# submission2019/cnn-quantization

Hardware: NVIDIA H100
Metric: resnet50_w4a4_images_per_s (higher is better)
Workload: dtype f32

## Files before the change

cnn-quantization_b200/_lib.py:

```python
import ctypes
import os

HERE = os.path.dirname(os.path.abspath(__file__))
LIB_PATH = os.environ.get("FQB200_LIB") or os.path.join(HERE, "libfqb200.so")

OK, ERR_INVALID, ERR_WORKSPACE, ERR_CUDA, ERR_UNSUPPORTED = 0, 1, 2, 3, 4
SCOPE_GROUP, SCOPE_GROUP_MEAN, SCOPE_TENSOR = 0, 1, 2
RANGE_MINMAX, RANGE_LAPLACE, RANGE_GAUS, RANGE_KSTD, RANGE_GIVEN = 0, 1, 2, 3, 4
LEAF_TORCH, LEAF_COMPILED, LEAF_MIDTREAD = 0, 1, 2
PRIOR_STD, PRIOR_B = 0, 1
STATS_STRIDE = 12
STAT_COLUMNS = ("min", "max", "mean", "b", "std", "delta", "offset", "bits", "scale", "zero_point", "qmax", "flags")

ABI_VERSION = 3


class Desc(ctypes.Structure):
    _fields_ = [
        ("outer", ctypes.c_int64), ("groups", ctypes.c_int64), ("inner", ctypes.c_int64),
        ("scope", ctypes.c_int32), ("range_mode", ctypes.c_int32), ("leaf", ctypes.c_int32),
        ("num_bits", ctypes.c_int32), ("positive", ctypes.c_int32), ("solve_f64", ctypes.c_int32),
        ("clip_k", ctypes.c_float),
        ("bit_alloc", ctypes.c_int32), ("bit_alloc_prior", ctypes.c_int32), ("bit_alloc_round", ctypes.c_int32),
        ("bit_alloc_target", ctypes.c_float),
        ("mt_target", ctypes.c_float), ("mt_clip", ctypes.c_int32),
        ("bias_corr", ctypes.c_int32), ("var_corr", ctypes.c_int32), ("stats_only", ctypes.c_int32),
        ("out_stats", ctypes.c_void_p),
        ("bias", ctypes.c_void_p),
        ("bias_period", ctypes.c_int64),
        ("channels_last", ctypes.c_int32),
        ("out_hist", ctypes.c_void_p),
        ("hist_bins", ctypes.c_int32), ("hist_offset", ctypes.c_int32),
        ("out_hist_clamped", ctypes.c_void_p),
        ("relu_passthrough", ctypes.c_int32),
        ("residual", ctypes.c_void_p), ("residual_relu", ctypes.c_int32),
        ("residual_stats", ctypes.c_void_p), ("residual_bias", ctypes.c_void_p),
        ("pool", ctypes.c_int32), ("pool_h", ctypes.c_int64), ("pool_w", ctypes.c_int64), ("pool_out", ctypes.c_void_p),
        ("given_delta", ctypes.c_void_p), ("given_offset", ctypes.c_void_p), ("given_bits", ctypes.c_void_p),
        ("debug_stamps", ctypes.c_void_p),
    ]


_vp, _i64, _i32, _f32, _sz, _desc = (ctypes.c_void_p, ctypes.c_int64, ctypes.c_int, ctypes.c_float, ctypes.c_size_t,
                                      ctypes.POINTER(Desc))
PROTOTYPES = {
    "fqb200_abi_version": (_i32, []),
    "fqb200_last_error": (ctypes.c_char_p, []),
    "fqb200_resident_ctas": (_i32, []),
    "fqb200_plan_info": (_i32, [_desc, ctypes.POINTER(ctypes.c_int64)]),
    "fqb200_selftest_division": (_i32, [_vp, _vp, _vp, _vp, _i64, _vp]),
    "fqb200_workspace_bytes": (_sz, [_desc]),
    "fqb200_workspace_init": (_i32, [_vp, _sz, _vp]),
    "fqb200_float2gemmlowp": (_i32, [_vp, _vp, _i64, _f32, _f32, _i32, _i32, _i32, _vp, _vp]),
    "fqb200_quantize1": (_i32, [_vp, _vp, _vp, _i64, _i64, _i64, _vp, _vp, _vp, _i32, _i32, _vp, _i32, _vp]),
    "fqb200_quantize1_bca": (_i32, [_vp, _vp, _i64, _i64, _i64, _vp, _vp, _vp, _i32, _i32, _vp, _i32, _vp, _vp, _sz, _vp]),
    "fqb200_fused": (_i32, [_desc, _vp, _vp, _vp, _sz, _vp]),
    "fqb200_fused_into": (_i32, [_desc, _vp, _vp, _i64, _vp, _sz, _vp]),
    "fqb200_add_relu": (_i32, [_vp, _vp, _vp, _i64, _vp]),
    "fqb200_maxpool2d_nhwc": (_i32, [_vp, _vp, _i64, _i64, _i64, _i64, _i32, _i32, _i32, _i32, _i32, _i32, _vp]),
    "fqb200_maxpool2d_nhwc_into": (_i32, [_vp, _vp, _i64, _i64, _i64, _i64, _i32, _i32, _i32, _i32, _i32, _i32, _i64, _vp]),
    "fqb200_kld_threshold": (_i32, [_vp, _i64, _i64, _i32, _i32, _vp, _vp, _vp, _vp, _sz, _vp]),
    "fqb200_kld_workspace_bytes": (_sz, [_i64, _i32]),
    "fqb200_sample_sumsq": (_i32, [_vp, _i64, _i64, _vp, _vp, _sz, _vp]),
    "fqb200_sample_sumsq_workspace_bytes": (_sz, [_i64, _i64]),
    "fqb200_clip_error": (_i32, [_vp, _i64, _i64, _i64, _i32, _vp, _i32, _i32, _i32, _i32, _vp, _vp, _vp, _sz, _i32, _vp]),
    "fqb200_clip_error_workspace_bytes": (_sz, [_i64, _i64, _i64, _i32]),
    "fqb200_clip_mse": (_i32, [_vp, _i64, _i64, _i64, _i32, _vp, _i32, _i32, _i32, _i32, _i32, _vp, _i32, _vp, _vp, _vp, _sz,
                               _i32, _vp]),
    "fqb200_clip_mse_widths": (_i32, [_vp, _i64, _i64, _i64, _i32, _vp, _i32, _i32, _i32, _i32, _i32, _vp, _vp, _i32, _vp, _vp,
                                      _vp, _sz, _i32, _vp]),
    "fqb200_clip_mse_workspace_bytes": (_sz, [_i64, _i64, _i64, _i32, _i32]),
    "fqb200_clip_mse_grid": (_i32, [_vp, _i64, _i64, _i64, _i32, _vp, _i32, _i32, _i32, _i32, _i32, _vp, _i32, _vp, _i32, _vp,
                                    _vp, _vp, _sz, _i32, _vp]),
    "fqb200_clip_mse_grid_workspace_bytes": (_sz, [_i64, _i64, _i64, _i32, _i32, _i32]),
    "fqb200_kmeans1d": (_i32, [_vp, _i64, _i32, _i64, _vp, _i32, _vp, _i32, _i64, _vp, _vp, _vp, _vp, _vp, _vp, _vp, _vp, _sz,
                               _i32, _vp]),
    "fqb200_kmeans1d_workspace_bytes": (_sz, [_i64, _i32]),
    "fqb200_sample_angles": (_i32, [_vp, _i64, _i64, _vp, _vp, _vp, _sz, _i32, _vp]),
    "fqb200_sample_angles_workspace_bytes": (_sz, [_i64, _i64]),
    "fqb200_sample_noise": (_i32, [_vp, _vp, _vp, _i64, _i64, _i64, _vp, _vp, _sz, _i32, _vp]),
    "fqb200_sample_noise_workspace_bytes": (_sz, [_i64, _i64]),
    "fqb200_quantize_weights_given": (_i32, [_vp, _vp, _i64, _i64, _vp, _vp, _vp, _i32, _i32, _i32, _vp, _vp, _sz, _vp]),
    "fqb200_quantize_weights_given_workspace_bytes": (_sz, [_i64, _i64, _i32, _i32, _i32, _i32]),
    "fqb200_allocate_widths": (_i32, [_vp, _i64, ctypes.c_double, _vp, _vp, _vp, _sz, _vp]),
    "fqb200_allocate_widths_workspace_bytes": (_sz, [_i64, ctypes.c_double]),
}
SYMBOLS = tuple(PROTOTYPES)


class FqError(RuntimeError):
    pass


_lib = None


def load():
    global _lib
    if _lib is not None:
        return _lib
    if not os.path.exists(LIB_PATH):
        raise FqError("libfqb200.so is not built (run `python cnn-quantization_b200/build.py` or "
                      "__graft_entry__.build()); there is no CPU fallback for the fake-quantization path")
    lib = ctypes.CDLL(LIB_PATH)
    for name, (restype, argtypes) in PROTOTYPES.items():
        fn = getattr(lib, name)
        fn.restype, fn.argtypes = restype, argtypes
    if lib.fqb200_abi_version() != ABI_VERSION:
        raise FqError("libfqb200.so ABI version mismatch")
    _lib = lib
    return lib


def check(rc):
    if rc != OK:
        raise FqError("fqb200 error %d: %s" % (rc, load().fqb200_last_error().decode()))
```

cnn-quantization_b200/csrc/fq_bulk.cuh:

```cuda
#pragma once
#include <cuda_runtime.h>
#include <stdint.h>

#include "fq_device.cuh"

namespace fqb {

constexpr int kConsumers = kThreads;
constexpr int kBulkThreads = kConsumers + 32;
constexpr int kConsumerWarps = kConsumers / 32;
#ifndef FQB_STAGE_VEC
#define FQB_STAGE_VEC 4
#endif
#ifndef FQB_STAGES
#define FQB_STAGES 6
#endif
#ifndef FQB_BULK_CTAS
#define FQB_BULK_CTAS 1
#endif
constexpr int kBulkCtasPerSm = FQB_BULK_CTAS;
constexpr int kStageVec = FQB_STAGE_VEC;
constexpr int kStages = FQB_STAGES;
constexpr unsigned kStageBytes = kStageVec * kConsumers * 16u;
#ifndef FQB_BULK_SPLIT
#define FQB_BULK_SPLIT 1
#endif
constexpr unsigned kBulkSplit = FQB_BULK_SPLIT;

__device__ __forceinline__ void consumer_sync() { cta_sync(); }

__device__ __forceinline__ unsigned smem_u32(const void* p) { return static_cast<unsigned>(__cvta_generic_to_shared(p)); }
__device__ __forceinline__ void mbar_init(unsigned bar, unsigned count) {
  asm volatile("mbarrier.init.shared::cta.b64 [%0], %1;" ::"r"(bar), "r"(count) : "memory");
}
__device__ __forceinline__ void mbar_fence_init() { asm volatile("fence.mbarrier_init.release.cluster;" ::: "memory"); }
__device__ __forceinline__ void mbar_arrive(unsigned bar) {
  asm volatile("{ .reg .b64 st; mbarrier.arrive.shared::cta.b64 st, [%0]; }" ::"r"(bar) : "memory");
}
__device__ __forceinline__ void mbar_arrive_expect_tx(unsigned bar, unsigned bytes) {
  asm volatile("{ .reg .b64 st; mbarrier.arrive.expect_tx.shared::cta.b64 st, [%0], %1; }" ::"r"(bar), "r"(bytes) : "memory");
}
__device__ __forceinline__ bool mbar_try_wait(unsigned bar, unsigned parity) {
  unsigned ok;
  asm volatile(
      "{ .reg .pred p; mbarrier.try_wait.parity.shared::cta.b64 p, [%1], %2; selp.u32 %0, 1, 0, p; }"
      : "=r"(ok)
      : "r"(bar), "r"(parity)
      : "memory");
  return ok != 0;
}
__device__ __forceinline__ void mbar_wait(unsigned bar, unsigned parity) {
  while (!mbar_try_wait(bar, parity)) {
  }
}
__device__ __forceinline__ void bulk_load_one(unsigned dst_smem, const void* src, unsigned bytes, unsigned bar) {
  asm volatile("cp.async.bulk.shared::cluster.global.mbarrier::complete_tx::bytes [%0], [%1], %2, [%3];" ::"r"(dst_smem),
               "l"(src), "r"(bytes), "r"(bar)
               : "memory");
}
__device__ __forceinline__ void bulk_load(unsigned dst_smem, const void* src, unsigned bytes, unsigned bar) {
  if (kBulkSplit == 1u) {
    bulk_load_one(dst_smem, src, bytes, bar);
    return;
  }
  constexpr unsigned piece = kStageBytes / kBulkSplit;
  for (unsigned off = 0; off < bytes; off += piece)
    bulk_load_one(dst_smem + off, static_cast<const unsigned char*>(src) + off, min(piece, bytes - off), bar);
}

struct FlatGeo {
  unsigned total_v;
  unsigned stride;
  unsigned stage_v;
  unsigned n_stages;
  unsigned unit_stages;
  unsigned units;
  unsigned channels;
  unsigned cv;
};

struct StageMeta {
  unsigned start;
  unsigned count;
  unsigned tag;
  unsigned pad;
};

struct BulkRing {
  alignas(8) unsigned long long full[kStages];
  alignas(8) unsigned long long empty[kStages];
  StageMeta meta[kStages];
  unsigned nstages;
};

struct RingPos {
  unsigned slot, parity, n;
  __device__ __forceinline__ void init(unsigned nstages = kStages) {
    slot = 0;
    parity = 0;
    n = nstages;
  }
  __device__ __forceinline__ void next() {
    if (++slot == n) {
      slot = 0;
      parity ^= 1u;
    }
  }
};

__device__ __forceinline__ void ring_init(BulkRing& r, unsigned nstages = kStages) {
  if (threadIdx.x == 0) {
    r.nstages = nstages;
#pragma unroll
    for (int s = 0; s < kStages; ++s) {
      mbar_init(smem_u32(&r.full[s]), 1u);
      mbar_init(smem_u32(&r.empty[s]), kConsumerWarps);
    }
    mbar_fence_init();
  }
  __syncthreads();
}

struct TicketPlan {
  unsigned nstatic;
  unsigned first, step;
  unsigned dyn_base;
};

constexpr unsigned kPairOffset = kStageBytes / 2u;

__device__ __forceinline__ FlatGeo half_geo(const FlatGeo& g) {
  FlatGeo h = g;
  h.stage_v = (kStageVec / 2u) * g.stride;
  h.n_stages = (g.total_v + h.stage_v - 1u) / h.stage_v;
  h.unit_stages = 2u * g.unit_stages;
  return h;
}

template <bool REV, bool PAIR = false>
__device__ __forceinline__ void produce_phase(const FlatGeo& g, const float4* src, unsigned* counter, const TicketPlan tp,
                                              BulkRing& r, unsigned char* stage_base, RingPos& pos,
                                              const float4* src2 = nullptr) {
  const unsigned total = g.units;
  unsigned k = 0;
  auto fetch = [&]() -> unsigned {
    unsigned long long t;
    if (k < tp.nstatic)
      t = tp.first + static_cast<unsigned long long>(k) * tp.step;
    else
      t = static_cast<unsigned long long>(tp.dyn_base) + atomicAdd(counter, 1u);
    ++k;
    return t < total ? static_cast<unsigned>(t) : 0xffffffffu;
  };
  unsigned cur = fetch();
  unsigned nxt = (cur != 0xffffffffu) ? fetch() : 0xffffffffu;
  while (cur != 0xffffffffu) {
    const unsigned nxt2 = (nxt != 0xffffffffu) ? fetch() : 0xffffffffu;
    const unsigned u = REV ? total - 1u - cur : cur;
    const unsigned g0 = u * g.unit_stages;
    const unsigned g1 = min(g0 + g.unit_stages, g.n_stages);
    for (unsigned i = g0; i < g1; ++i) {
      const unsigned st = REV ? g1 - 1u - (i - g0) : i;
      const unsigned start = st * g.stage_v;
      const unsigned count = min(g.stage_v, g.total_v - start);
      mbar_wait(smem_u32(&r.empty[pos.slot]), pos.parity ^ 1u);
      r.meta[pos.slot].start = start;
      r.meta[pos.slot].count = count;
      r.meta[pos.slot].tag = 0u;
      const unsigned bar = smem_u32(&r.full[pos.slot]);
      mbar_arrive_expect_tx(bar, PAIR ? count * 32u : count * 16u);
      bulk_load(smem_u32(stage_base + pos.slot * kStageBytes), src + start, count * 16u, bar);
      if (PAIR) bulk_load(smem_u32(stage_base + pos.slot * kStageBytes + kPairOffset), src2 + start, count * 16u, bar);
      pos.next();
    }
    cur = nxt;
    nxt = nxt2;
  }
  mbar_wait(smem_u32(&r.empty[pos.slot]), pos.parity ^ 1u);
  r.meta[pos.slot].start = 0u;
  r.meta[pos.slot].count = 0u;
  mbar_arrive(smem_u32(&r.full[pos.slot]));
  pos.next();
}

struct RowsGeo {
  unsigned rows, row_v;
  unsigned stages_per_row;
  unsigned units_per_row;
};

__device__ __forceinline__ RowsGeo half_rows(const FlatGeo& h, const RowsGeo& rg) {
  RowsGeo r = rg;
  r.stages_per_row = (rg.row_v + h.stage_v - 1u) / h.stage_v;
  r.units_per_row = (r.stages_per_row + h.unit_stages - 1u) / h.unit_stages;
  return r;
}

template <bool REV, bool PAIR = false>
__device__ __forceinline__ void produce_rows_phase(const FlatGeo& g, const RowsGeo& rg, const float4* src, unsigned* counter,
                                                   const TicketPlan tp, BulkRing& r, unsigned char* stage_base, RingPos& pos,
                                                   const float4* src2 = nullptr) {
  const unsigned total = g.units;
  unsigned k = 0;
  auto fetch = [&]() -> unsigned {
    unsigned long long t;
    if (k < tp.nstatic)
      t = tp.first + static_cast<unsigned long long>(k) * tp.step;
    else
      t = static_cast<unsigned long long>(tp.dyn_base) + atomicAdd(counter, 1u);
    ++k;
    return t < total ? static_cast<unsigned>(t) : 0xffffffffu;
  };
  unsigned cur = fetch();
  unsigned nxt = (cur != 0xffffffffu) ? fetch() : 0xffffffffu;
  while (cur != 0xffffffffu) {
    const unsigned nxt2 = (nxt != 0xffffffffu) ? fetch() : 0xffffffffu;
    const unsigned u = REV ? total - 1u - cur : cur;
    const unsigned row = u / rg.units_per_row;
    const unsigned part = u - row * rg.units_per_row;
    const unsigned s0 = part * g.unit_stages;
    const unsigned s1 = min(s0 + g.unit_stages, rg.stages_per_row);
    for (unsigned i = s0; i < s1; ++i) {
      const unsigned st = REV ? s1 - 1u - (i - s0) : i;
      const unsigned off = st * g.stage_v;
      const unsigned start = row * rg.row_v + off;
      const unsigned count = min(g.stage_v, rg.row_v - off);
      mbar_wait(smem_u32(&r.empty[pos.slot]), pos.parity ^ 1u);
      r.meta[pos.slot].start = start;
      r.meta[pos.slot].count = count;
      r.meta[pos.slot].tag = row | (i + 1u == s1 ? 0x80000000u : 0u);
      const unsigned bar = smem_u32(&r.full[pos.slot]);
      mbar_arrive_expect_tx(bar, PAIR ? count * 32u : count * 16u);
      bulk_load(smem_u32(stage_base + pos.slot * kStageBytes), src + start, count * 16u, bar);
      if (PAIR) bulk_load(smem_u32(stage_base + pos.slot * kStageBytes + kPairOffset), src2 + start, count * 16u, bar);
      pos.next();
    }
    cur = nxt;
    nxt = nxt2;
  }
  mbar_wait(smem_u32(&r.empty[pos.slot]), pos.parity ^ 1u);
  r.meta[pos.slot].start = 0u;
  r.meta[pos.slot].count = 0u;
  r.meta[pos.slot].tag = 0u;
  mbar_arrive(smem_u32(&r.full[pos.slot]));
  pos.next();
// ... 272 lines not shown
```

cnn-quantization_b200/csrc/fq_cl.cuh:

```cuda
#pragma once

namespace fqb {

__device__ __forceinline__ unsigned enc_ordered(float x) {
  const unsigned b = __float_as_uint(x);
  return (b & 0x80000000u) ? ~b : (b | 0x80000000u);
}
__device__ __forceinline__ float dec_ordered(unsigned e) {
  return __uint_as_float((e & 0x80000000u) ? (e & 0x7fffffffu) : ~e);
}

constexpr unsigned kAccU = 2u * kMaxNhwcChannels;
constexpr unsigned kAccD = 3u * kMaxNhwcChannels;

struct ClView {
  unsigned* amin_inv;
  unsigned* amax;
  double* asum;
  double* asq;
  double* aabs;
};
__device__ __forceinline__ ClView cl_view(const FusedArgs& A, unsigned bank) {
  ClView v;
  v.amin_inv = A.amin_inv + bank * kAccU;
// ... 553 lines not shown
  cl_combine_add_f64(cx.cbuf, g.cv, g.stride, s2.sa, acc.aabs + rb, s2.sa, nullptr, s2.sa, nullptr);
}

template <int LEAF, bool HIST>
__device__ __noinline__ void cl_phase_apply(const FusedArgs& A, ClCtx& cx, const LeafParam (&lp)[4], unsigned* hist) {
  const FlatGeo& g = *cx.g;
  const unsigned t = threadIdx.x;
  if (HIST) {
    for (unsigned i = t; i < kHistWords; i += kConsumers) hist[i] = 0u;
    consumer_sync();
  }
  ClApply<LEAF, HIST> ap{A, hist};
  ap.init(cx.c0, cx.active, lp);
  RingPos pos = cx.pos;
  if (A.pool.tiles) {
    if (A.pool.kind == 3u)
      consume_pool3_phase(g, A.pool, *cx.ring, cx.stages, pos, ap);
    else
      consume_pool_phase(g, A.pool, *cx.ring, cx.stages, pos, ap);
  } else if (A.residual) {
    const FlatGeo h = half_geo(g);
    consume_pair_phase(h, *cx.ring, cx.stages, pos, ap);
  } else {
    consume_phase(g, *cx.ring, cx.stages, pos, ap);
  }
  cx.pos = pos;
  if (HIST) {
    consumer_sync();
    const unsigned bins = static_cast<unsigned>(A.hist_bins);
    const unsigned copies = max(1u, min(static_cast<unsigned>(kWarps), kHistWords / bins));
    for (unsigned b = t; b < bins; b += kConsumers) {
      unsigned long long cnt = 0;
      for (unsigned w = 0; w < copies; ++w) cnt += hist[w * bins + b];
      if (cnt) atomicAdd(A.hist + b, cnt);
    }
    if (LEAF == FQB200_LEAF_MIDTREAD && A.hist_clamped && cx.active) {
#pragma unroll
      for (int i = 0; i < 4; ++i) {
        if (ap.nlo[i]) atomicAdd(A.hist_clamped + 2u * (cx.c0 + i), static_cast<unsigned long long>(ap.nlo[i]));
        if (ap.nhi[i]) atomicAdd(A.hist_clamped + 2u * (cx.c0 + i) + 1u, static_cast<unsigned long long>(ap.nhi[i]));
      }
    }
  }
}

constexpr unsigned kClStagingBytes = 4u * kConsumers * 8u;
constexpr unsigned kClTableChannels = 1024;
constexpr unsigned kClCombineBytes = kClStagingBytes + kClTableChannels * 4u;

template <int LEAF, bool DEV, bool HIST>
__global__ void __launch_bounds__(kBulkThreads, kBulkCtasPerSm) fq_cl_kernel(const __grid_constant__ FusedArgs A) {
  extern __shared__ __align__(128) unsigned char fq_dyn[];
  unsigned char* stages = fq_dyn;
  unsigned char* cbuf = fq_dyn + kStages * kStageBytes;
  float* tab_mean = reinterpret_cast<float*>(cbuf + kClStagingBytes);
  unsigned* hist = reinterpret_cast<unsigned*>(stages + (kStages - 1) * kStageBytes);
  __shared__ BulkRing ring;
  __shared__ LeaderSmem lsm;
  __shared__ alignas(8) unsigned long long solver_done;
  const FlatGeo& g = A.flat;
  const unsigned C = g.channels, cv = g.cv;
  const unsigned launch = ld_ws(&A.sync->launch_count);
  const unsigned bank = launch & 1u;
  const unsigned tag = launch + 1u;
  const bool alloc = (LEAF == FQB200_LEAF_MIDTREAD) || (A.bit_alloc && A.num_bits <= 4);
  const bool aux_needs_b = alloc && LEAF != FQB200_LEAF_MIDTREAD && A.prior == FQB200_PRIOR_B;
  const bool solver_in_s2 = alloc && !aux_needs_b && DEV && gridDim.x > 1u;
  __shared__ alignas(8) unsigned long long phase_go[2];
  if (threadIdx.x == 0) {
    mbar_init(smem_u32(&solver_done), 1u);
    mbar_init(smem_u32(&phase_go[0]), 1u);
    mbar_init(smem_u32(&phase_go[1]), 1u);
  }
  const unsigned nstages = HIST ? kStages - 1u : kStages;
  ring_init(ring, nstages);

  if (threadIdx.x >= kConsumers) {
    if (threadIdx.x == kConsumers) {
      RingPos pos;
      pos.init(nstages);
      const float4* src = reinterpret_cast<const float4*>(A.in);
      const TicketPlan all = {2u, blockIdx.x, gridDim.x, 2u * gridDim.x};
      const TicketPlan no0 = {blockIdx.x == 0 ? 0u : 2u, blockIdx.x - 1u, gridDim.x - 1u, 2u * (gridDim.x - 1u)};
      produce_phase<false>(g, src, &A.sync->unit_counter[0], all, ring, stages, pos);
      if (DEV) {
        mbar_wait(smem_u32(&phase_go[0]), 0u);
        if (solver_in_s2 && blockIdx.x == 0) mbar_wait(smem_u32(&solver_done), 0u);
        produce_phase<true>(g, src, &A.sync->unit_counter[1], solver_in_s2 ? no0 : all, ring, stages, pos);
      }
      if (!A.stats_only) {
        mbar_wait(smem_u32(&phase_go[1]), 0u);
        if (A.pool.tiles && A.pool.kind == 3u)
          produce_pool3_phase(g, A.pool, src, &A.sync->unit_counter[2], all, ring, stages, pos);
        else if (A.pool.tiles)
          produce_pool_phase(g, A.pool, src, &A.sync->unit_counter[2], all, ring, stages, pos);
        else if (A.residual)
          produce_phase<!DEV, true>(half_geo(g), src, &A.sync->unit_counter[2], all, ring, stages, pos,
                                    reinterpret_cast<const float4*>(A.residual));
        else
          produce_phase<!DEV>(g, src, &A.sync->unit_counter[2], all, ring, stages, pos);
      }
    }
    return;
  }

  const unsigned t = threadIdx.x;
  const bool active = t < g.stride;
  const bool direct = cv == g.stride;
  const unsigned col = active ? t % cv : 0u;
  const unsigned c0 = 4u * col;
  const double n = A.n_per_group;
  const ClView acc = cl_view(A, bank);
  const unsigned rep = A.nhwc_rep;
  const unsigned rep_base = (blockIdx.x % rep) * C;
  unsigned epoch = 0;
  if (blockIdx.x == 0) stamp(A, 0);

  if (blockIdx.x == gridDim.x - 1u) {
    const ClView other = cl_view(A, bank ^ 1u);
    uint4* zu = reinterpret_cast<uint4*>(other.amin_inv);
    uint4* zd = reinterpret_cast<uint4*>(other.asum);
    const uint4 z = make_uint4(0u, 0u, 0u, 0u);
    for (unsigned i = t; i < kAccU / 4u; i += kConsumers) zu[i] = z;
    for (unsigned i = t; i < kAccD / 2u; i += kConsumers) zd[i] = z;
  }

  ClCtx cx;
  cx.g = &g;
  cx.ring = &ring;
  cx.stages = stages;
  cx.cbuf = cbuf;
  cx.pos.init(nstages);
  cx.acc = acc;
  cx.rep_base = rep_base;
  cx.c0 = c0;
  cx.active = active;
  float kshift[4];
  cl_phase_s1(A, cx, kshift);
  if (t == 0) mbar_arrive(smem_u32(&phase_go[DEV ? 0 : 1]));
  if (blockIdx.x == 0) stamp(A, 1);
  grid_barrier_cl(A.sync, epoch);
  if (blockIdx.x == 0) stamp(A, 4);

  float mean[4];
  if (direct) {
#pragma unroll
    for (int i = 0; i < 4; ++i)
      mean[i] = static_cast<float>(cl_mean(acc, rep, C, c0 + i, kshift[i], (A.bias && active) ? __ldg(A.bias + c0 + i) : 0.f, n));
  } else {
    for (unsigned c = t; c < C; c += kConsumers)
      tab_mean[c] = static_cast<float>(cl_mean(acc, rep, C, c, ld_tensor(A.in + c), A.bias ? __ldg(A.bias + c) : 0.f, n));
    consumer_sync();
#pragma unroll
    for (int i = 0; i < 4; ++i) mean[i] = tab_mean[c0 + i];
  }

  if (alloc && !aux_needs_b && blockIdx.x == 0) {
    cl_solve_aux(A, acc, lsm, tag, false, !solver_in_s2);
    stamp(A, 12);
    if (t == 0) mbar_arrive(smem_u32(&solver_done));
  }

  if constexpr (DEV) {
    cl_phase_s2(A, cx, mean);
    if (t == 0) mbar_arrive(smem_u32(&phase_go[1]));
    if (blockIdx.x == 0) stamp(A, 5);
    grid_barrier_cl(A.sync, epoch);
    if (blockIdx.x == 0) stamp(A, 8);
    if (aux_needs_b && blockIdx.x == 0) cl_solve_aux(A, acc, lsm, tag, true, true);
  }
  if (alloc && !solver_in_s2) {
    if (t == 0)
      while (ld_acquire_u32(&A.sync->aux_ready) != tag) __nanosleep(40);
    consumer_sync();
  }

  LeafParam lp[4];
  const bool do_export = A.out_stats != nullptr && blockIdx.x == 0;
  if (direct) {
#pragma unroll
    for (int i = 0; i < 4; ++i) lp[i] = cl_channel_param<LEAF, DEV>(A, acc, rep, C, c0 + i, mean[i], n, alloc, do_export && active);
  } else {
    LeafParam* tab_lp = reinterpret_cast<LeafParam*>(cbuf);
// ... 612 lines not shown
```

cnn-quantization_b200/csrc/fqb200.cu:

```cuda
#include <cuda_runtime.h>
#include <math.h>
#include <stdint.h>
#include <stdio.h>
#include <stdlib.h>
#include <string.h>

#include "../../include/fqb200.h"
#include "fq_device.cuh"
#include "fq_bulk.cuh"

namespace fqb {

__constant__ float kGaus[9] = {0.f, 1.24f, 1.71f, 2.15f, 2.55f, 2.93f, 3.28f, 3.61f, 3.92f};
__constant__ float kGausPos[9] = {0.f, 1.71f, 2.15f, 2.55f, 2.93f, 3.28f, 3.61f, 3.92f, 4.2f};
__constant__ float kLaplace[9] = {1.05f, 1.86f, 2.83f, 3.89f, 5.03f, 6.2f, 7.41f, 8.64f, 9.89f};
__constant__ float kLaplacePos[9] = {1.86f, 2.83f, 3.89f, 5.02f, 6.2f, 7.41f, 8.64f, 9.89f, 11.16f};
constexpr int kTable = 101;
__constant__ double kOmegaTable[kTable];
__constant__ double kAlphaTable[kTable];

enum : int { FLAG_PASSTHROUGH = 1, FLAG_TRUE_ZERO = 2, FLAG_RELU = 4 };

struct alignas(16) LeafParam {
  float a, b, c;
// ... 1380 lines not shown

struct Plan {
  fqb::Geometry geo;
  fqb::FlatGeo flat;
  int vec;
  int mode;
  int grid;
};

constexpr uint64_t kUnitsPerCta = 8;

int make_plan(int64_t outer, int64_t groups, int64_t inner, bool can_vec, bool allow_bundle, int max_ctas, Plan* pl) {
  if (outer <= 0 || groups <= 0 || inner <= 0) return fail(FQB200_ERR_INVALID, "non-positive tensor extent%s");
  if (groups > 0x3fffffffLL || outer > 0x7fffffffLL || inner > 0x7fffffffLL * 4LL)
    return fail(FQB200_ERR_UNSUPPORTED, "tensor extent exceeds 2^31%s");
  int vec = (can_vec && inner % 4 == 0) ? 4 : 1;
  int mode = vec;
  uint64_t bundle = 1;
  if (vec == 1 && can_vec && allow_bundle && inner >= 4) {
    const uint64_t b = (inner % 2 == 0) ? 2 : 4;
    const uint64_t row_v = b * static_cast<uint64_t>(inner) / 4;
    if (groups % b == 0 && row_v <= static_cast<uint64_t>(fqb::kThreads)) {
      bundle = b;
      vec = 4;
      mode = 8;
    }
  }
  const uint64_t G = static_cast<uint64_t>(groups) / bundle;
  const uint64_t inner_v = bundle * static_cast<uint64_t>(inner) / vec;
  if (inner_v > 0xffffffffULL) return fail(FQB200_ERR_UNSUPPORTED, "row too long%s");
  const uint64_t stride = (mode == 8) ? (fqb::kThreads / inner_v) * inner_v : fqb::kThreads;
  const uint64_t group_v = static_cast<uint64_t>(outer) * inner_v;
  const uint64_t total_v = group_v * G;
  if (total_v >= (1ULL << 32)) return fail(FQB200_ERR_UNSUPPORTED, "tensors of 2^32 vectors (64 GB) and more are not supported%s");
  const uint64_t ctas = static_cast<uint64_t>(max_ctas);
  const uint64_t min_unit_v = static_cast<uint64_t>(fqb::kRingDepth) * stride;
  uint64_t parts = (kUnitsPerCta * ctas + G - 1) / G;
  const uint64_t max_parts = group_v / min_unit_v > 0 ? group_v / min_unit_v : 1;
  if (parts > max_parts) parts = max_parts;
  if (parts < 1) parts = 1;
  while ((group_v + parts - 1) / parts >= 0x7fffffffULL) ++parts;
  uint64_t part_v = (group_v + parts - 1) / parts;
  if (mode == 8) part_v = (part_v + inner_v - 1) / inner_v * inner_v;
  parts = (group_v + part_v - 1) / part_v;
  if (parts * G >= 0xfffffff0ULL) return fail(FQB200_ERR_UNSUPPORTED, "too many work units%s");
  const uint64_t units = parts * G;
  unsigned lanes = 32;
  while (lanes > 1 && (static_cast<uint64_t>(fqb::kThreads / lanes) < static_cast<uint64_t>(groups) || (lanes >> 1) >= parts)) lanes >>= 1;
  fqb::Geometry& g = pl->geo;
  g.groups = static_cast<unsigned>(G);
  g.channels = static_cast<unsigned>(groups);
  g.bundle = static_cast<unsigned>(bundle);
  g.stride = static_cast<unsigned>(stride);
  g.parts = static_cast<unsigned>(parts);
  g.units = static_cast<unsigned>(units);
  g.inner_v = static_cast<unsigned>(inner_v);
  g.step_q = static_cast<unsigned>(stride / inner_v);
  g.step_r = static_cast<unsigned>(stride % inner_v);
  g.red_lanes = lanes;
  g.part_v = static_cast<unsigned>(part_v);
  g.group_v = group_v;
  g.row_pitch = G * inner_v;
  pl->vec = vec;
  pl->mode = mode;
  pl->grid = grid_for(units, ctas);
  return FQB200_OK;
}

bool flat_eligible(int64_t channels) { return channels % 4 == 0 && channels / 4 >= 1 && channels / 4 <= fqb::kConsumers; }

int make_plan_flat(uint64_t elems, int64_t channels, int max_ctas, Plan* pl) {
  if (elems == 0 || elems % 4 != 0) return fail(FQB200_ERR_UNSUPPORTED, "flat stream needs a multiple of 4 elements%s");
  const uint64_t total_v = elems / 4;
  if (total_v >= (1ULL << 32)) return fail(FQB200_ERR_UNSUPPORTED, "tensors of 2^32 vectors (64 GB) and more are not supported%s");
  const uint64_t cv = channels > 0 ? static_cast<uint64_t>(channels) / 4 : 1;
  if (channels > 0 && !flat_eligible(channels)) return fail(FQB200_ERR_UNSUPPORTED, "channels-last needs C %% 4 == 0 and C <= 2048%s");
  const uint64_t stride = (fqb::kConsumers / cv) * cv;
  const uint64_t stage_v = static_cast<uint64_t>(fqb::kStageVec) * stride;
  const uint64_t n_stages = (total_v + stage_v - 1) / stage_v;
  const uint64_t ctas = static_cast<uint64_t>(max_ctas);
  uint64_t unit_stages = n_stages / (kUnitsPerCta * ctas);
  if (unit_stages < 2) unit_stages = 2;
  if (unit_stages > 64) unit_stages = 64;
  const uint64_t units = (n_stages + unit_stages - 1) / unit_stages;
  fqb::FlatGeo& g = pl->flat;
  g.total_v = static_cast<unsigned>(total_v);
  g.stride = static_cast<unsigned>(stride);
  g.stage_v = static_cast<unsigned>(stage_v);
  g.n_stages = static_cast<unsigned>(n_stages);
  g.unit_stages = static_cast<unsigned>(unit_stages);
  g.units = static_cast<unsigned>(units);
  g.channels = static_cast<unsigned>(channels > 0 ? channels : 0);
  g.cv = static_cast<unsigned>(cv);
  memset(&pl->geo, 0, sizeof(pl->geo));
  pl->geo.channels = g.channels;
  pl->vec = 4;
  pl->mode = 2;
  pl->grid = grid_for(units, ctas);
  return FQB200_OK;
}

int make_plan_rows(uint64_t rows, uint64_t row_elems, int64_t channels, int max_ctas, Plan* pl, fqb::RowsGeo* rg) {
  if (rows == 0 || row_elems == 0 || row_elems % 4 != 0 || rows > fqb::kMaxNhwcChannels)
    return fail(FQB200_ERR_UNSUPPORTED, "row stream needs rows <= 4096 of a multiple of 4 elements%s");
  const uint64_t row_v = row_elems / 4;
  if (rows * row_v >= (1ULL << 32)) return fail(FQB200_ERR_UNSUPPORTED, "tensors of 2^32 vectors (64 GB) and more are not supported%s");
  const uint64_t cv = channels > 0 ? static_cast<uint64_t>(channels) / 4 : 1;
  if (channels > 0 && (!flat_eligible(channels) || row_v % cv != 0)) return fail(FQB200_ERR_UNSUPPORTED, "bias period does not fit the rows%s");
  const uint64_t stride = (fqb::kConsumers / cv) * cv;
  const uint64_t stage_v = static_cast<uint64_t>(fqb::kStageVec) * stride;
  const uint64_t spr = (row_v + stage_v - 1) / stage_v;
  const uint64_t ctas = static_cast<uint64_t>(max_ctas);
  uint64_t unit_stages = rows * spr / (kUnitsPerCta * ctas);
  if (unit_stages < 1) unit_stages = 1;
  if (unit_stages > 64) unit_stages = 64;
  if (unit_stages > spr) unit_stages = spr;
  const uint64_t upr = (spr + unit_stages - 1) / unit_stages;
  const uint64_t units = rows * upr;
  if (units >= 0xfffffff0ULL) return fail(FQB200_ERR_UNSUPPORTED, "too many work units%s");
  fqb::FlatGeo& g = pl->flat;
  g.total_v = static_cast<unsigned>(rows * row_v);
  g.stride = static_cast<unsigned>(stride);
  g.stage_v = static_cast<unsigned>(stage_v);
  g.n_stages = static_cast<unsigned>(rows * spr);
  g.unit_stages = static_cast<unsigned>(unit_stages);
  g.units = static_cast<unsigned>(units);
  g.channels = static_cast<unsigned>(channels > 0 ? channels : 0);
  g.cv = static_cast<unsigned>(cv);
  rg->rows = static_cast<unsigned>(rows);
  rg->row_v = static_cast<unsigned>(row_v);
  rg->stages_per_row = static_cast<unsigned>(spr);
  rg->units_per_row = static_cast<unsigned>(upr);
  memset(&pl->geo, 0, sizeof(pl->geo));
  pl->geo.channels = static_cast<unsigned>(rows);
  pl->vec = 4;
  pl->mode = 3;
  pl->grid = grid_for(units, ctas);
  return FQB200_OK;
}

bool rows_supported(const fqb200_desc* d, bool can_vec) {
  if (d->leaf != FQB200_LEAF_COMPILED || d->range_mode != FQB200_RANGE_MINMAX || d->bias_corr || d->var_corr || d->channels_last ||
      d->out_hist || !can_vec || d->outer != 1 || d->inner % 4 != 0 || d->groups > static_cast<int64_t>(fqb::kMaxNhwcChannels))
    return false;
  if (!(d->scope == FQB200_SCOPE_GROUP_MEAN || d->scope == FQB200_SCOPE_TENSOR || d->groups == 1)) return false;
  if (d->bias) {
    if (d->bias_period >= 0) return false;
    const int64_t c = -d->bias_period;
    if (!flat_eligible(c) || d->inner % c != 0) return false;
  }
  return true;
}

size_t align_up(size_t v, size_t a) { return (v + a - 1) / a * a; }

size_t kld_workspace(int64_t rows, int num_bins) {
  return align_up(static_cast<size_t>(rows) * 4, 256) + static_cast<size_t>(rows) * static_cast<size_t>(num_bins) * 4;
}

size_t sums_workspace(int64_t rows, int64_t row_len, int sums) {
  const unsigned long long chunk = fqb::sums_chunk(static_cast<unsigned long long>(row_len));
  const unsigned long long chunks = (static_cast<unsigned long long>(row_len) + chunk - 1) / chunk;
  return chunks > 1 ? static_cast<size_t>(rows) * static_cast<size_t>(chunks) * static_cast<size_t>(sums) * 8 : 0;
}

template <int S>
int launch_sums(const float* y, const float* q, const float* bias, int64_t bias_period, int64_t rows, int64_t row_len,
                double* out, void* workspace, int32_t max_ctas, void* stream, const char* what) {
  using namespace fqb;
  DeviceInfo* di = nullptr;
  const int rc = get_device(&di);
  if (rc != FQB200_OK) return rc;
  cudaStream_t st = static_cast<cudaStream_t>(stream);
  SumsArgs A;
  memset(&A, 0, sizeof(A));
  A.y = y;
  A.q = q;
  A.bias = bias;
  A.period = static_cast<unsigned>(bias_period < 0 ? 0ull - static_cast<unsigned long long>(bias_period)
                                                   : static_cast<unsigned long long>(bias_period));
  A.rows = static_cast<unsigned long long>(rows);
  A.row_len = static_cast<unsigned long long>(row_len);
  A.chunk = sums_chunk(A.row_len);
  A.chunks = (A.row_len + A.chunk - 1) / A.chunk;
  A.partial = static_cast<double*>(workspace);
  A.out = out;
  const int grid = grid_for(A.rows * A.chunks, di->sms * (2048ull / kSumsThreads), max_ctas);
  const bool vec = row_len % 4 == 0 && aligned16(y) && (!q || aligned16(q));
#define FQB_LAUNCH_SUMS(B)                                                          \
  do {                                                                              \
    if (vec) fq_sums_partial_kernel<4, S, B><<<grid, kSumsThreads, 0, st>>>(A);     \
    else     fq_sums_partial_kernel<1, S, B><<<grid, kSumsThreads, 0, st>>>(A);     \
  } while (0)
  if constexpr (S == 1) FQB_LAUNCH_SUMS(kSumsBiasNone);
  else if (!bias) FQB_LAUNCH_SUMS(kSumsBiasNone);
  else if (bias_period > 0) FQB_LAUNCH_SUMS(kSumsBiasNchw);
  else FQB_LAUNCH_SUMS(kSumsBiasCl);
#undef FQB_LAUNCH_SUMS
  if (A.chunks > 1) {
    const unsigned long long blocks = (A.rows * S + kSumsThreads - 1) / kSumsThreads;
    fq_sums_finish_kernel<S><<<static_cast<unsigned>(blocks), kSumsThreads, 0, st>>>(A);
  }
  return launched(what);
}

size_t angle_workspace(int64_t rows, int64_t row_len) {
  const fqb::AngleSplit s = fqb::angle_split(static_cast<unsigned long long>(rows), static_cast<unsigned long long>(row_len));
  return static_cast<size_t>(s.pairs * s.slices) * fqb::kAngTile * fqb::kAngTile * 8;
}

unsigned long long cliperr_units_per_group(int64_t outer, int64_t inner, int channels_last) {
// ... 301 lines not shown
                   (alloc && d->bit_alloc_prior == FQB200_PRIOR_B) || d->stats_only || d->out_stats != nullptr;
      fp->kernel = cl_kernel_ptr(d->leaf, A.need_dev != 0, d->out_hist != nullptr);
      fp->smem = cl_smem(d->out_hist != nullptr);
      fp->name = "fq_cl_kernel";
    } else {
      A.nhwc_rep = 1;
      A.need_dev = (d->range_mode != FQB200_RANGE_MINMAX) || alloc || d->var_corr || d->leaf == FQB200_LEAF_MIDTREAD || d->stats_only;
      fp->slots = static_cast<uint64_t>(pl.geo.parts) * pl.geo.channels;
      fp->kernel = A.bias_magic ? reinterpret_cast<const void*>(fqb::fq_fused_kernel<4, FQB200_LEAF_COMPILED, false, false, true>)
                                : fused_kernel_ptr(pl.mode, d->leaf, A.need_dev != 0, d->bias_corr || d->var_corr);
      fp->block = fqb::kThreads;
      fp->smem = dyn_smem(pl.vec);
      fp->name = "fq_fused_kernel";
    }
  }
  fp->workspace = carve(nullptr, fp->slots, pl.geo.channels, nullptr);
  return FQB200_OK;
}

DeviceInfo plan_residency() {
  DeviceInfo* di = nullptr;
  if (get_device(&di) == FQB200_OK) return *di;
  DeviceInfo h;
  h.resident = kAssumedSms * fqb::kCtasPerSm;
  h.resident_cl[0] = h.resident_cl[1] = h.resident_rows = kAssumedSms * fqb::kBulkCtasPerSm;
  return h;
}

}

extern "C" {

int fqb200_abi_version(void) { return FQB200_ABI_VERSION; }

const char* fqb200_last_error(void) { return g_err; }

int fqb200_resident_ctas(void) {
  DeviceInfo* di = nullptr;
  if (get_device(&di) != FQB200_OK) return -1;
  return di->resident;
}

size_t fqb200_workspace_bytes(const fqb200_desc* d) {
  if (check_desc(d) != FQB200_OK) return 0;
  if (d->outer == 0 || d->groups == 0 || d->inner == 0) return 256;
  const DeviceInfo r = plan_residency();
  size_t bytes = 0;
  for (bool can_vec : {false, true}) {
    FusedPlan fp;
    if (plan_fused(d, can_vec, 0, r, &fp) != FQB200_OK) continue;
    const size_t need = fp.workspace ? fp.workspace : 256;
    if (need > bytes) bytes = need;
  }
  return bytes;
}

int fqb200_workspace_init(void* workspace, size_t bytes, void* stream) {
  const size_t head = carve(nullptr, 0, 0, nullptr);
  if (!workspace || bytes < head) return fail(FQB200_ERR_WORKSPACE, "workspace too small%s");
  cudaError_t e = cudaMemsetAsync(workspace, 0, head, static_cast<cudaStream_t>(stream));
  if (e != cudaSuccess) return fail(FQB200_ERR_CUDA, "cudaMemsetAsync: %s", cudaGetErrorString(e));
  return FQB200_OK;
}

int fqb200_plan_info(const fqb200_desc* d, int64_t* out8) {
  g_err[0] = 0;
  int rc = check_desc(d);
  if (rc != FQB200_OK) return rc;
  if (!out8) return fail(FQB200_ERR_INVALID, "null output%s");
  FusedPlan fp;
  rc = plan_fused(d, true, 0, plan_residency(), &fp);
  if (rc != FQB200_OK) return rc;
  const Plan& pl = fp.pl;
  if (pl.mode == 2 || pl.mode == 3) {
    out8[0] = pl.mode; out8[1] = pl.grid; out8[2] = pl.flat.units; out8[3] = pl.flat.unit_stages; out8[4] = pl.flat.stage_v;
    out8[5] = pl.flat.stride; out8[6] = fqb::kStages; out8[7] = d->range_mode == FQB200_RANGE_GIVEN ? 1 : 2 + fp.A.need_dev;
    return FQB200_OK;
  }
  out8[0] = pl.mode; out8[1] = pl.grid; out8[2] = pl.geo.units; out8[3] = pl.geo.parts; out8[4] = pl.geo.part_v;
  out8[5] = pl.geo.stride; out8[6] = fqb::kRingDepth; out8[7] = pl.geo.red_lanes;
  return FQB200_OK;
}

int fqb200_float2gemmlowp(const float* in, float* out, int64_t n, float range, float offset, int num_bits, int int_exp,
                          int enforce_true_zero, const float* noise, void* stream) {
  g_err[0] = 0;
  if (n < 0 || num_bits < 1 || num_bits > 30) return fail(FQB200_ERR_INVALID, "bad n / num_bits%s");
  if (n == 0) return FQB200_OK;
  if (!in || !out) return fail(FQB200_ERR_INVALID, "null tensor pointer%s");
  cudaStream_t st = static_cast<cudaStream_t>(stream);
  if (range <= 0) {
    if (in != out) {
      cudaError_t e = cudaMemcpyAsync(out, in, static_cast<size_t>(n) * sizeof(float), cudaMemcpyDeviceToDevice, st);
      if (e != cudaSuccess) return fail(FQB200_ERR_CUDA, "cudaMemcpyAsync: %s", cudaGetErrorString(e));
    }
    return FQB200_OK;
  }
  DeviceInfo* di = nullptr;
  int rc = get_device(&di);
  if (rc != FQB200_OK) return rc;
  const long long qmax_i = (1ll << num_bits) - 1;
  volatile float scale = range / static_cast<float>(qmax_i);
  if (int_exp) scale = powf(2.f, static_cast<float>(static_cast<int>(ceilf(log2f(scale)))));
  volatile float zr = -offset / scale;
  const float zero_point = roundf(zr);
  fqb::LeafParam q;
  q.a = scale;
  q.b = enforce_true_zero ? zero_point : -offset;
  q.c = static_cast<float>(qmax_i);
  q.flags = enforce_true_zero ? fqb::FLAG_TRUE_ZERO : 0;
  const bool vec = (n % 4 == 0) && aligned16(in) && aligned16(out) && (!noise || aligned16(noise));
  if (vec && static_cast<uint64_t>(n) >= (1ull << 20) && static_cast<uint64_t>(n) / 4 < (1ull << 32)) {
    Plan pl;
    rc = make_plan_flat(static_cast<uint64_t>(n), 0, di->resident_cl[0] * 2, &pl);
    if (rc != FQB200_OK) return rc;
    fqb::LeafBulkArgs B;
    B.flat = pl.flat;
    B.in = in;
    B.out = out;
    B.noise = noise;
    B.q = q;
    if (noise) fqb::fq_leaf_bulk_kernel<true><<<pl.grid, fqb::kBulkThreads, cl_given_smem(), st>>>(B);
    else       fqb::fq_leaf_bulk_kernel<false><<<pl.grid, fqb::kBulkThreads, cl_given_smem(), st>>>(B);
    return launched("fq_leaf_bulk_kernel");
  }
  const unsigned long long nvec = vec ? static_cast<unsigned long long>(n / 4) : static_cast<unsigned long long>(n);
  const int grid = grid_for((nvec + fqb::kThreads * 4ull - 1) / (fqb::kThreads * 4ull), di->resident * 2ull);
  const float as = fabsf(q.a);
  const bool fast = (as > 1e-30f) && (as < 1e30f);
#define FQB_LAUNCH_LEAF(V, N, F) fqb::fq_leaf_kernel<V, N, F><<<grid, fqb::kThreads, 0, st>>>(in, out, noise, nvec, q)
  if (vec) {
    if (noise) { if (fast) FQB_LAUNCH_LEAF(4, true, true); else FQB_LAUNCH_LEAF(4, true, false); }
    else       { if (fast) FQB_LAUNCH_LEAF(4, false, true); else FQB_LAUNCH_LEAF(4, false, false); }
  } else {
    if (noise) { if (fast) FQB_LAUNCH_LEAF(1, true, true); else FQB_LAUNCH_LEAF(1, true, false); }
    else       { if (fast) FQB_LAUNCH_LEAF(1, false, true); else FQB_LAUNCH_LEAF(1, false, false); }
  }
#undef FQB_LAUNCH_LEAF
  return launched("fq_leaf_kernel");
}

int fqb200_quantize1(const float* in, float* out, float* grid, int64_t outer, int64_t groups, int64_t inner,
                     const float* delta, const float* offset, const float* bits, int per_group, int num_bits,
                     const float* bias, int channels_last, void* stream) {
  g_err[0] = 0;
  if (outer == 0 || groups == 0 || inner == 0) return FQB200_OK;
  if (!in || !out || !delta || !offset) return fail(FQB200_ERR_INVALID, "null pointer%s");
  if (num_bits < 1 || num_bits > 8) {
    if (!bits) return fail(FQB200_ERR_INVALID, "num_bits must be in 1..8%s");
  }
  if (bits && !per_group) return fail(FQB200_ERR_INVALID, "per-row bit widths need per-group parameters%s");
  DeviceInfo* di = nullptr;
  int rc = get_device(&di);
  if (rc != FQB200_OK) return rc;
  Plan pl;
  const bool can_vec = aligned16(in) && aligned16(out) && (!grid || aligned16(grid));
  fqb::FusedArgs A;
  memset(&A, 0, sizeof(A));
  A.in = in;
  A.out = out;
  A.grid_out = grid;
  A.leaf = FQB200_LEAF_TORCH;
  A.num_bits = num_bits;
  A.g_delta = delta;
  A.g_offset = offset;
  A.g_bits = bits;
// ... 723 lines not shown
```

include/fqb200.h:

```cpp
#ifndef FQB200_H_
#define FQB200_H_

#include <stddef.h>
#include <stdint.h>

#ifdef __cplusplus
extern "C" {
#endif

#define FQB200_ABI_VERSION 3

#define FQB200_OK 0
#define FQB200_ERR_INVALID 1
#define FQB200_ERR_WORKSPACE 2
#define FQB200_ERR_CUDA 3
#define FQB200_ERR_UNSUPPORTED 4

#define FQB200_SCOPE_GROUP 0
#define FQB200_SCOPE_GROUP_MEAN 1
#define FQB200_SCOPE_TENSOR 2
#define FQB200_RANGE_MINMAX 0
#define FQB200_RANGE_LAPLACE 1
#define FQB200_RANGE_GAUS 2
#define FQB200_RANGE_KSTD 3
#define FQB200_RANGE_GIVEN 4
#define FQB200_LEAF_TORCH 0
#define FQB200_LEAF_COMPILED 1
#define FQB200_LEAF_MIDTREAD 2
#define FQB200_PRIOR_STD 0
#define FQB200_PRIOR_B 1

#define FQB200_STATS_STRIDE 12

typedef struct fqb200_desc {
  int64_t outer, groups, inner;
  int32_t scope;
  int32_t range_mode;
  int32_t leaf;
  int32_t num_bits;
  int32_t positive;
  int32_t solve_f64;
  float clip_k;
  int32_t bit_alloc;
  int32_t bit_alloc_prior;
  int32_t bit_alloc_round;
  float bit_alloc_target;
  float mt_target;
  int32_t mt_clip;
  int32_t bias_corr;
  int32_t var_corr;
  int32_t stats_only;
  float* out_stats;
  const float* bias;
  int64_t bias_period;
  int32_t channels_last;
  unsigned long long* out_hist;
  int32_t hist_bins;
  int32_t hist_offset;
  unsigned long long* out_hist_clamped;
  int32_t relu_passthrough;
  const float* residual;
  int32_t residual_relu;
  const float* residual_stats;
  const float* residual_bias;
  int32_t pool;
  int64_t pool_h, pool_w;
  float* pool_out;
  const float* given_delta;
  const float* given_offset;
  const float* given_bits;
  unsigned long long* debug_stamps;
} fqb200_desc;

int fqb200_abi_version(void);
const char* fqb200_last_error(void);
int fqb200_resident_ctas(void);

int fqb200_plan_info(const fqb200_desc* d, int64_t* out8);
int fqb200_selftest_division(const float* a, const float* b, float* fast, float* ieee, int64_t n, void* stream);

size_t fqb200_workspace_bytes(const fqb200_desc* d);
int fqb200_workspace_init(void* workspace, size_t bytes, void* stream);

int fqb200_float2gemmlowp(const float* in, float* out, int64_t n, float range, float offset, int num_bits,
                          int int_exp, int enforce_true_zero, const float* noise, void* stream);

int fqb200_quantize1(const float* in, float* out, float* grid, int64_t outer, int64_t groups, int64_t inner,
                     const float* delta, const float* offset, const float* bits, int per_group, int num_bits,
                     const float* bias, int channels_last, void* stream);

int fqb200_quantize1_bca(const float* in, float* out, int64_t outer, int64_t groups, int64_t inner, const float* delta,
                         const float* offset, const float* bits, int per_group, int num_bits, const float* bias, int relu_first,
                         float* out_qbias, void* workspace, size_t workspace_bytes, void* stream);

int fqb200_maxpool2d_nhwc(const float* in, float* out, int64_t n, int64_t h, int64_t w, int64_t c, int kh, int kw, int sh, int sw,
                          int ph, int pw, void* stream);
int fqb200_maxpool2d_nhwc_into(const float* in, float* out, int64_t n, int64_t h, int64_t w, int64_t c, int kh, int kw,
                               int sh, int sw, int ph, int pw, int64_t out_pixel_stride, void* stream);

int fqb200_add_relu(const float* a, const float* b, float* out, int64_t n, void* stream);

int fqb200_fused(const fqb200_desc* d, const float* in, float* out, void* workspace, size_t workspace_bytes,
                 void* stream);
int fqb200_fused_into(const fqb200_desc* d, const float* in, float* out, int64_t out_pixel_stride, void* workspace,
                      size_t workspace_bytes, void* stream);

int fqb200_kld_threshold(const float* in, int64_t rows, int64_t row_len, int num_bins, int num_quantized_bins, float* out_th,
                         float* out_div, int32_t* out_idx, void* workspace, size_t workspace_bytes, void* stream);
size_t fqb200_kld_workspace_bytes(int64_t rows, int num_bins);

int fqb200_sample_sumsq(const float* in, int64_t rows, int64_t row_len, double* out, void* workspace, size_t workspace_bytes,
                        void* stream);
size_t fqb200_sample_sumsq_workspace_bytes(int64_t rows, int64_t row_len);

int fqb200_sample_angles(const float* in, int64_t rows, int64_t row_len, float* out_angles, double* out_gram,
                         void* workspace, size_t workspace_bytes, int32_t max_ctas, void* stream);
size_t fqb200_sample_angles_workspace_bytes(int64_t rows, int64_t row_len);

int fqb200_sample_noise(const float* y, const float* q, const float* bias, int64_t bias_period, int64_t rows, int64_t row_len,
                        double* out, void* workspace, size_t workspace_bytes, int32_t max_ctas, void* stream);
size_t fqb200_sample_noise_workspace_bytes(int64_t rows, int64_t row_len);

int fqb200_clip_error(const float* in, int64_t outer, int64_t groups, int64_t inner, int32_t channels_last, const float* stats,
                      int32_t num_bits, int32_t positive, int32_t bit_alloc, int32_t solve_f64, double* out, float* out_params,
                      void* workspace, size_t workspace_bytes, int32_t max_ctas, void* stream);
size_t fqb200_clip_error_workspace_bytes(int64_t outer, int64_t groups, int64_t inner, int32_t channels_last);

int fqb200_clip_mse(const float* in, int64_t outer, int64_t groups, int64_t inner, int32_t channels_last, const float* stats,
                    int32_t num_bits, int32_t positive, int32_t bit_alloc, int32_t solve_f64, int32_t prior,
                    const float* multipliers, int32_t num_multipliers, double* out, float* out_params, void* workspace,
                    size_t workspace_bytes, int32_t max_ctas, void* stream);
int fqb200_clip_mse_widths(const float* in, int64_t outer, int64_t groups, int64_t inner, int32_t channels_last,
                           const float* stats, int32_t num_bits, int32_t positive, int32_t bit_alloc, int32_t solve_f64,
                           int32_t prior, const float* multipliers, const int32_t* widths, int32_t num_multipliers,
                           double* out, float* out_params, void* workspace, size_t workspace_bytes, int32_t max_ctas,
                           void* stream);
size_t fqb200_clip_mse_workspace_bytes(int64_t outer, int64_t groups, int64_t inner, int32_t channels_last,
                                       int32_t num_multipliers);
int fqb200_clip_mse_grid(const float* in, int64_t outer, int64_t groups, int64_t inner, int32_t channels_last,
                         const float* stats, int32_t num_bits, int32_t positive, int32_t bit_alloc, int32_t solve_f64,
                         int32_t prior, const float* multipliers, int32_t num_multipliers, const int32_t* widths,
                         int32_t num_widths, double* out, float* out_params, void* workspace, size_t workspace_bytes,
                         int32_t max_ctas, void* stream);
size_t fqb200_clip_mse_grid_workspace_bytes(int64_t outer, int64_t groups, int64_t inner, int32_t channels_last,
                                            int32_t num_multipliers, int32_t num_widths);

#define FQB200_KMEANS_NONE 0
#define FQB200_KMEANS_QUANTIZE 1
#define FQB200_KMEANS_CLIP 2
int fqb200_kmeans1d(const float* in, int64_t n, int32_t num_bits, int64_t first_id, const double* draws, int32_t n_trials,
                    const double* init, int32_t task, int64_t rows, uint8_t* out_labels, float* out_centres,
                    double* out_inertia, int32_t* out_n_iter, int64_t* out_init_ids, float* out, float* out_bcorr,
                    void* workspace, size_t workspace_bytes, int32_t max_ctas, void* stream);
size_t fqb200_kmeans1d_workspace_bytes(int64_t n, int32_t k);

int fqb200_quantize_weights_given(const float* in, float* out, int64_t groups, int64_t inner, const float* delta,
                                  const float* offset, const float* bits, int32_t num_bits, int32_t bias_corr,
                                  int32_t var_corr, unsigned long long* hist, void* workspace, size_t workspace_bytes,
                                  void* stream);
size_t fqb200_quantize_weights_given_workspace_bytes(int64_t groups, int64_t inner, int32_t num_bits, int32_t has_bits,
                                                     int32_t bias_corr, int32_t var_corr);
// ... 9 lines not shown
```

Before: 9018.

## Add tiered tail units to flat-stream work split and flip phase walk direction

Splits the end of the flat stage stream into tiers of geometrically shrinking work units (2×CTAs units per tier) so dynamic ticket scheduling finishes with small pieces, reducing tail imbalance across CTAs. Unit-to-stage mapping moves into a shared host/device helper, reverse traversal is redefined over stage positions, and the forward/reverse order of the phases is swapped so each phase starts where the previous one ended, for better L2 reuse. It adds a host-side plan_walk query for inspecting spans, and costs more units and tickets plus slightly more index arithmetic per unit.

```diff
diff --git a/cnn-quantization_b200/_lib.py b/cnn-quantization_b200/_lib.py
--- a/cnn-quantization_b200/_lib.py
+++ b/cnn-quantization_b200/_lib.py
@@ -48,6 +48,7 @@
     "fqb200_last_error": (ctypes.c_char_p, []),
     "fqb200_resident_ctas": (_i32, []),
     "fqb200_plan_info": (_i32, [_desc, ctypes.POINTER(ctypes.c_int64)]),
+    "fqb200_plan_walk": (_i32, [_desc, _i32, ctypes.POINTER(ctypes.c_int64), _i64]),
     "fqb200_selftest_division": (_i32, [_vp, _vp, _vp, _vp, _i64, _vp]),
     "fqb200_workspace_bytes": (_sz, [_desc]),
     "fqb200_workspace_init": (_i32, [_vp, _sz, _vp]),
diff --git a/cnn-quantization_b200/csrc/fq_bulk.cuh b/cnn-quantization_b200/csrc/fq_bulk.cuh
--- a/cnn-quantization_b200/csrc/fq_bulk.cuh
+++ b/cnn-quantization_b200/csrc/fq_bulk.cuh
@@ -77,7 +77,35 @@
   unsigned units;
   unsigned channels;
   unsigned cv;
-};
+  unsigned tail_start;
+  unsigned tail_units;
+  unsigned tail_tiers;
+  unsigned tail_min;
+};
+
+struct UnitSpan {
+  unsigned p0, p1;
+};
+__host__ __device__ __forceinline__ UnitSpan unit_span(const FlatGeo& g, unsigned u) {
+  const unsigned bulk = (g.tail_start + g.unit_stages - 1u) / g.unit_stages;
+  unsigned p0, len, end;
+  if (u < bulk) {
+    p0 = u * g.unit_stages;
+    len = g.unit_stages;
+    end = g.tail_start < g.n_stages ? g.tail_start : g.n_stages;
+  } else {
+    u -= bulk;
+    p0 = g.tail_start;
+    len = g.tail_min << (g.tail_tiers - 1u - u / g.tail_units);
+    for (unsigned s = g.tail_min << (g.tail_tiers - 1u); s > len; s >>= 1) p0 += g.tail_units * s;
+    p0 += (u % g.tail_units) * len;
+    end = g.n_stages;
+  }
+  UnitSpan r;
+  r.p0 = p0;
+  r.p1 = p0 + len < end ? p0 + len : end;
+  return r;
+}
 
 struct StageMeta {
   unsigned start;
@@ -129,11 +157,13 @@
 
 constexpr unsigned kPairOffset = kStageBytes / 2u;
 
-__device__ __forceinline__ FlatGeo half_geo(const FlatGeo& g) {
+__host__ __device__ __forceinline__ FlatGeo half_geo(const FlatGeo& g) {
   FlatGeo h = g;
   h.stage_v = (kStageVec / 2u) * g.stride;
   h.n_stages = (g.total_v + h.stage_v - 1u) / h.stage_v;
   h.unit_stages = 2u * g.unit_stages;
+  h.tail_start = 2u * g.tail_start;
+  h.tail_min = 2u * g.tail_min;
   return h;
 }
 
@@ -156,11 +186,9 @@
   unsigned nxt = (cur != 0xffffffffu) ? fetch() : 0xffffffffu;
   while (cur != 0xffffffffu) {
     const unsigned nxt2 = (nxt != 0xffffffffu) ? fetch() : 0xffffffffu;
-    const unsigned u = REV ? total - 1u - cur : cur;
-    const unsigned g0 = u * g.unit_stages;
-    const unsigned g1 = min(g0 + g.unit_stages, g.n_stages);
-    for (unsigned i = g0; i < g1; ++i) {
-      const unsigned st = REV ? g1 - 1u - (i - g0) : i;
+    const UnitSpan us = unit_span(g, cur);
+    for (unsigned p = us.p0; p < us.p1; ++p) {
+      const unsigned st = REV ? g.n_stages - 1u - p : p;
       const unsigned start = st * g.stage_v;
       const unsigned count = min(g.stage_v, g.total_v - start);
       mbar_wait(smem_u32(&r.empty[pos.slot]), pos.parity ^ 1u);
diff --git a/cnn-quantization_b200/csrc/fq_cl.cuh b/cnn-quantization_b200/csrc/fq_cl.cuh
--- a/cnn-quantization_b200/csrc/fq_cl.cuh
+++ b/cnn-quantization_b200/csrc/fq_cl.cuh
@@ -659,11 +659,11 @@
       const float4* src = reinterpret_cast<const float4*>(A.in);
       const TicketPlan all = {2u, blockIdx.x, gridDim.x, 2u * gridDim.x};
       const TicketPlan no0 = {blockIdx.x == 0 ? 0u : 2u, blockIdx.x - 1u, gridDim.x - 1u, 2u * (gridDim.x - 1u)};
-      produce_phase<false>(g, src, &A.sync->unit_counter[0], all, ring, stages, pos);
+      produce_phase<true>(g, src, &A.sync->unit_counter[0], all, ring, stages, pos);
       if (DEV) {
         mbar_wait(smem_u32(&phase_go[0]), 0u);
         if (solver_in_s2 && blockIdx.x == 0) mbar_wait(smem_u32(&solver_done), 0u);
-        produce_phase<true>(g, src, &A.sync->unit_counter[1], solver_in_s2 ? no0 : all, ring, stages, pos);
+        produce_phase<false>(g, src, &A.sync->unit_counter[1], solver_in_s2 ? no0 : all, ring, stages, pos);
       }
       if (!A.stats_only) {
         mbar_wait(smem_u32(&phase_go[1]), 0u);
@@ -672,10 +672,10 @@
         else if (A.pool.tiles)
           produce_pool_phase(g, A.pool, src, &A.sync->unit_counter[2], all, ring, stages, pos);
         else if (A.residual)
-          produce_phase<!DEV, true>(half_geo(g), src, &A.sync->unit_counter[2], all, ring, stages, pos,
-                                    reinterpret_cast<const float4*>(A.residual));
+          produce_phase<DEV, true>(half_geo(g), src, &A.sync->unit_counter[2], all, ring, stages, pos,
+                                   reinterpret_cast<const float4*>(A.residual));
         else
-          produce_phase<!DEV>(g, src, &A.sync->unit_counter[2], all, ring, stages, pos);
+          produce_phase<DEV>(g, src, &A.sync->unit_counter[2], all, ring, stages, pos);
       }
     }
     return;
diff --git a/cnn-quantization_b200/csrc/fqb200.cu b/cnn-quantization_b200/csrc/fqb200.cu
--- a/cnn-quantization_b200/csrc/fqb200.cu
+++ b/cnn-quantization_b200/csrc/fqb200.cu
@@ -1486,7 +1486,10 @@
   uint64_t unit_stages = n_stages / (kUnitsPerCta * ctas);
   if (unit_stages < 2) unit_stages = 2;
   if (unit_stages > 64) unit_stages = 64;
-  const uint64_t units = (n_stages + unit_stages - 1) / unit_stages;
+  const uint64_t tiers = unit_stages > 2 ? 63 - __builtin_clzll(unit_stages) : 0;
+  const uint64_t tail_units = tiers ? 2 * ctas : 0;
+  const uint64_t tail_start = n_stages - tail_units * ((1ULL << tiers) - 1);
+  const uint64_t units = (tail_start + unit_stages - 1) / unit_stages + tiers * tail_units;
   fqb::FlatGeo& g = pl->flat;
   g.total_v = static_cast<unsigned>(total_v);
   g.stride = static_cast<unsigned>(stride);
@@ -1496,6 +1499,10 @@
   g.units = static_cast<unsigned>(units);
   g.channels = static_cast<unsigned>(channels > 0 ? channels : 0);
   g.cv = static_cast<unsigned>(cv);
+  g.tail_start = static_cast<unsigned>(tail_start);
+  g.tail_units = static_cast<unsigned>(tail_units);
+  g.tail_tiers = static_cast<unsigned>(tiers);
+  g.tail_min = 1;
   memset(&pl->geo, 0, sizeof(pl->geo));
   pl->geo.channels = g.channels;
   pl->vec = 4;
@@ -1531,6 +1538,10 @@
   g.units = static_cast<unsigned>(units);
   g.channels = static_cast<unsigned>(channels > 0 ? channels : 0);
   g.cv = static_cast<unsigned>(cv);
+  g.tail_start = g.n_stages;
+  g.tail_units = 0;
+  g.tail_tiers = 0;
+  g.tail_min = 1;
   rg->rows = static_cast<unsigned>(rows);
   rg->row_v = static_cast<unsigned>(row_v);
   rg->stages_per_row = static_cast<unsigned>(spr);
@@ -1998,6 +2009,25 @@
   return FQB200_OK;
 }
 
+int fqb200_plan_walk(const fqb200_desc* d, int pair, int64_t* spans, int64_t cap) {
+  g_err[0] = 0;
+  int rc = check_desc(d);
+  if (rc != FQB200_OK) return rc;
+  if (!spans) return fail(FQB200_ERR_INVALID, "null output%s");
+  FusedPlan fp;
+  rc = plan_fused(d, true, 0, plan_residency(), &fp);
+  if (rc != FQB200_OK) return rc;
+  if (fp.pl.mode != 2) return fail(FQB200_ERR_INVALID, "not a flat-stream launch%s");
+  const fqb::FlatGeo g = pair ? fqb::half_geo(fp.pl.flat) : fp.pl.flat;
+  if (cap < 2 * static_cast<int64_t>(g.units)) return fail(FQB200_ERR_INVALID, "spans holds fewer than 2 * units values%s");
+  for (unsigned u = 0; u < g.units; ++u) {
+    const fqb::UnitSpan us = fqb::unit_span(g, u);
+    spans[2 * u] = us.p0;
+    spans[2 * u + 1] = us.p1;
+  }
+  return FQB200_OK;
+}
+
 int fqb200_float2gemmlowp(const float* in, float* out, int64_t n, float range, float offset, int num_bits, int int_exp,
                           int enforce_true_zero, const float* noise, void* stream) {
   g_err[0] = 0;
diff --git a/include/fqb200.h b/include/fqb200.h
--- a/include/fqb200.h
+++ b/include/fqb200.h
@@ -77,6 +77,7 @@
 int fqb200_resident_ctas(void);
 
 int fqb200_plan_info(const fqb200_desc* d, int64_t* out8);
+int fqb200_plan_walk(const fqb200_desc* d, int pair, int64_t* spans, int64_t cap);
 int fqb200_selftest_division(const float* a, const float* b, float* fast, float* ieee, int64_t n, void* stream);
 
 size_t fqb200_workspace_bytes(const fqb200_desc* d);
```

After: 9060 (median of 6 runs). Within noise of the previous version (+0.5%).
